# brunoasm/varKoder

Measured on AMD Instinct MI355X. Metric: Gbases/s for `varKoder image` k=7, 150 bp reads, higher is better.
Workload: dtype u32

## Files before the change

varkoder_amd/csrc/vk_count.h:

```cpp
#ifndef VK_COUNT_H
#define VK_COUNT_H

#include <hip/hip_runtime.h>

#include <cstdint>

#include "vk_lane.h"

namespace {

constexpr int kWaves = 16;
constexpr int kCountThreads = kWaves * 64;
constexpr int kPiece = 4096;
constexpr uint32_t kMaxBins = 16384;
#ifndef VK_K1_OCC
#define VK_K1_OCC 8
#endif
#ifndef VK_K1_PF
#define VK_K1_PF 2
#endif


__device__ __forceinline__ uint32_t nl_flags(uint32_t w) {
    uint32_t z = w ^ 0x0A0A0A0Au;
// ... 728 lines not shown
        const uint32_t pos = have ? static_cast<uint32_t>(__builtin_ctzll(m)) : 0u;
        m &= m - 1ull;
        const uint32_t ph = (lph + t) & 3u;
        const bool anchor = have && ph == 0u;
        if (have && ph == 1u) acc += static_cast<long long>(blk + pos);
        if (anchor) acc -= static_cast<long long>(blk + pos) + 1ll;
        const unsigned long long am = __ballot(anchor);
        if (am != 0ull) {
            const uint32_t na = static_cast<uint32_t>(__builtin_popcountll(am));
            if (nanch + na > cap) full = true;
            else if (anchor) seg[nanch + static_cast<uint32_t>(__builtin_popcountll(am & ((1ull << ln) - 1ull)))] = static_cast<uint32_t>(blk + pos);
            if (!full) nanch += na;
        }
        ++t;
    }
}


#ifdef VK_DIAG_NO_DSADD
#define VK_DSADD(a) "s_nop 0\n\t"
#else
#define VK_DSADD(a) "ds_add_u32 " a ", %17\n\t"
#endif
template <int K>
__device__ __forceinline__ void windows_lds1(uint32_t ch, uint32_t C, uint32_t ok, uint32_t lds_base,
                                             uint32_t& probe_addr, unsigned long long& probe_mask) {
    static_assert(2 * K + 2 <= 16, "paired extraction needs the field << 2 to fit 16 bits");
    constexpr uint32_t kMask4 = ((1u << (2 * K)) - 1u) << 2;
    const uint32_t one = 1u;
    uint32_t w = vkl::lshl_or(vkl::alignbit(ok, ok, 16u), 1u, ok);
#pragma unroll
    for (int half = 0; half < 2; ++half) {
        uint32_t a[8];
#pragma unroll
        for (int j = 0; j < 4; ++j) {
            const int i = 15 - 4 * half - j;
            const int plo = i - 8;
            const int o = 30 + 2 * (plo - K + 1);
            const int word = o >> 5, sh = o & 31;
            uint32_t x;
            if (word == 1) x = sh == 0 ? C : (C >> sh);
            else x = vkl::alignbit(C, ch, static_cast<uint32_t>(sh));
            a[2 * j] = (x & kMask4) + lds_base;
            a[2 * j + 1] = ((x >> 16) & kMask4) + lds_base;
        }
        unsigned long long m0, m1, m2, m3, m4, m5, m6, m7;
        const unsigned long long exec_in = __builtin_amdgcn_read_exec();
        asm volatile(
            "v_add_co_u32_e64 %0, %1, %0, %0\n\t"
            "v_add_co_u32_e64 %0, %2, %0, %0\n\t"
            "v_add_co_u32_e64 %0, %3, %0, %0\n\t"
            "v_add_co_u32_e64 %0, %4, %0, %0\n\t"
            "v_add_co_u32_e64 %0, %5, %0, %0\n\t"
            "v_add_co_u32_e64 %0, %6, %0, %0\n\t"
            "v_add_co_u32_e64 %0, %7, %0, %0\n\t"
            "v_add_co_u32_e64 %0, %8, %0, %0\n\t"
            "s_mov_b64 exec, %1\n\t" VK_DSADD("%9") 
            "s_mov_b64 exec, %2\n\t" VK_DSADD("%10") 
            "s_mov_b64 exec, %3\n\t" VK_DSADD("%11") 
            "s_mov_b64 exec, %4\n\t" VK_DSADD("%12") 
            "s_mov_b64 exec, %5\n\t" VK_DSADD("%13") 
            "s_mov_b64 exec, %6\n\t" VK_DSADD("%14") 
            "s_mov_b64 exec, %7\n\t" VK_DSADD("%15") 
            "s_mov_b64 exec, %8\n\t" VK_DSADD("%16") 
            "s_mov_b64 exec, %18"
            : "+v"(w), "=&s"(m0), "=&s"(m1), "=&s"(m2), "=&s"(m3), "=&s"(m4), "=&s"(m5), "=&s"(m6), "=&s"(m7)
            : "v"(a[0]), "v"(a[1]), "v"(a[2]), "v"(a[3]), "v"(a[4]), "v"(a[5]), "v"(a[6]), "v"(a[7]), "v"(one), "s"(exec_in)
            : "memory");
        if (half == 1) {
            probe_addr = a[7];
            probe_mask = m7;
        }
    }
}

struct GeneralState {
    uint32_t ctx_c, ctx_bad, pph, hot, tick;
    uint32_t nanch, full, sites;
};



template <int K, bool INDEX>
__device__ __attribute__((noinline)) GeneralState general_piece(uint4 q0, uint4 q1, uint4 q2, uint4 q3, GeneralState st,
                                                                uint32_t packed, uint32_t* hist, uint32_t hist_base,
                                                                uint32_t* iseg, uint32_t icap, uint32_t iblk) {
    const uint32_t flags = packed & 3u, ph0 = (packed >> 2) & 3u, ivalid = packed >> 4;
    const int lane = static_cast<int>(lane_now());
    const uint32_t d[16] = {q0.x, q0.y, q0.z, q0.w, q1.x, q1.y, q1.z, q1.w, q2.x, q2.y, q2.z, q2.w, q3.x, q3.y, q3.z, q3.w};
    const bool first = (flags & 1u) != 0u, has_pre = (flags & 2u) != 0u;
    uint32_t pph = st.pph;
    vkl::LaneBits lb;
    const uint32_t c = __any(vkl::has_non_ascii(d)) ? vkl::classify<false>(d, lb) : vkl::classify<true>(d, lb);
    const uint32_t incl = wave_inclusive_sum(c);
    const uint32_t total = lane_bcast(incl, 63);
    if (first) pph = has_pre ? ph0 - lane_bcast(c, 0) : 0u;
    const uint32_t lph = (pph + incl - c) & 3u;
    vkl::Mask128 seq;
    const bool degenerate = __any(c > 4u);
    uint32_t s_raw = 0;
    const bool four = !degenerate && __any(c > 3u);
    if (degenerate) seq = vkl::seq_mask_general(lb.NL, lph);
    else if (four) seq = vkl::seq_mask_fast4(lb.NL, lph, vkl::ones_below, vkl::ones_not_below, s_raw);
    else seq = vkl::seq_mask_count(lb.NL, lph);
    uint32_t bad[4], ok[4];
    vkl::bad_mask(lb, seq, bad);
    const uint32_t badh = wave_prev_lane(bad[3], st.ctx_bad);
    const uint32_t ch = wave_prev_lane(lb.C[3], st.ctx_c);
    st.ctx_bad = lane_bcast(bad[3], 63);
    st.ctx_c = lane_bcast(lb.C[3], 63);
    vkl::ok_mask<K>(badh, bad, ok);
    if (first && lane == 0 && has_pre) { ok[0] = 0u; ok[1] = 0u; ok[2] = 0u; ok[3] = 0u; }
    if constexpr (INDEX) {
        const bool mine = !(first && lane == 0 && has_pre);
        uint32_t mlo, mhi;
        {
            uint32_t v[8];
#pragma unroll
            for (int j = 0; j < 8; ++j) v[j] = vkl::udot4(nl_flags(d[2 * j + 1]), 0x80402010u, vkl::udot4(nl_flags(d[2 * j]), 0x08040201u, 0u));
            mlo = (v[0] >> 7) | (v[1] << 1) | (v[2] << 9) | (v[3] << 17);
            mhi = (v[4] >> 7) | (v[5] << 1) | (v[6] << 9) | (v[7] << 17);
        }
        bool full = false;
        long long unused = 0;
        uint32_t nanch = st.nanch;
        index_block(mlo, mhi, lph, static_cast<uint64_t>(iblk) + 64u * static_cast<uint32_t>(lane), mine, iseg, icap, nanch, full, unused);
        st.nanch = nanch;
        st.full = full ? 1u : 0u;
        uint32_t sites = 0;
        const int vb = static_cast<int>(ivalid) - 64 * lane;
#pragma unroll
        for (int g = 0; g < 4; ++g) {
            const int vg = vb - 16 * g;
            const uint32_t inside = vg >= 16 ? 0xFFFFFFFFu : (vg <= 0 ? 0u : ((1u << (2 * vg)) - 1u));
            sites += vkl::popc(seq.w[g] & ~lb.NL[g] & inside & 0x55555555u);
        }
        st.sites = mine ? sites : 0u;
    }
    uint32_t pa;
    unsigned long long pm;
    uint32_t still = 0;
    uint32_t tick = st.tick & 0x7FFFFFFFu;
    if (st.hot == 0u) windows_lds<K>(ch, lb.C, ok, hist_base, pa, pm);
    else {
        ++tick;
        uint4* const xb = reinterpret_cast<uint4*>(hist + (1u << (2 * K))) + (threadIdx.x >> 6) * 64u;
        still = windows_lds_hot<K>(ch, lb.C, ok, hist, hist_base, lane, (st.tick >> 31) == 0u || (tick & 7u) == 0u, pa, pm, xb);
    }
    st.hot = (still != 0u || probe_low_complexity(pa, pm, tick)) ? 1u : 0u;
    st.tick = (tick & 0x7FFFFFFFu) | (still == 2u ? 0x80000000u : 0u);
    st.pph = pph + total;
    __builtin_amdgcn_s_waitcnt(0xC07F);
    return st;
}

constexpr uint32_t kSetAside = 6;
constexpr uint32_t kSetAsideBatch = 21;

template <int K, bool INDEX>
__global__ __launch_bounds__(kCountThreads, 8) void vk_aside_kernel(const uint8_t* __restrict__ fastq, const uint64_t* __restrict__ offs,
                                                                     const uint64_t* __restrict__ lens, uint32_t nsamples, uint32_t parts,
                                                                     uint32_t* __restrict__ hist_out, const uint32_t* __restrict__ aside,
                                                                     uint32_t aside_cap, const uint32_t* __restrict__ aside_n, IndexParams ip,
                                                                     uint32_t upb) {
    typedef uint32_t u32x4 __attribute__((ext_vector_type(4)));
    constexpr uint32_t NCODE = 1u << (2 * K);
    constexpr bool LDSH = NCODE <= kMaxBins;
    __shared__ uint32_t lhist[LDSH ? NCODE : 1];
    __shared__ uint32_t any_list;
    const uint32_t ablocks = (parts + upb - 1u) / upb;
    const uint32_t smp = blockIdx.x / ablocks;
    const uint32_t part0 = (blockIdx.x % ablocks) * upb, part1 = part0 + upb < parts ? part0 + upb : parts;
    const uint32_t tid = threadIdx.x;
    const uint32_t wave = static_cast<uint32_t>(__builtin_amdgcn_readfirstlane(static_cast<int>(tid >> 6)));
    if (tid == 0) any_list = 0u;
    __syncthreads();
    {
        uint32_t any = 0u;
        for (uint32_t part = part0; part < part1; ++part) any |= aside_n[(smp * parts + part) * kWaves + wave];
        if (any != 0u && (tid & 63u) == 0u) any_list = 1u;
    }
    __syncthreads();
    if (any_list == 0u) return;
    if constexpr (LDSH) {
        for (uint32_t i = tid; i < NCODE; i += kCountThreads) lhist[i] = 0u;
        __syncthreads();
    }
    const uint32_t lhist_base = static_cast<uint32_t>(reinterpret_cast<uintptr_t>((__attribute__((address_space(3))) uint32_t*)lhist));
    const uint8_t* sbase = fastq + offs[smp];
    uint32_t* hist = hist_out + static_cast<uint64_t>(smp) * NCODE;
    const uint32_t lane = tid & 63u;
    const uint32_t ent = lane / 3u, j = lane - 3u * ent;
    for (uint32_t part = part0; part < part1; ++part) {
    const uint32_t unit = smp * parts + part;
    const uint32_t gw = unit * kWaves + wave;
    const uint32_t naside = aside_n[gw];
    const WaveRange wr = wave_range(lens[smp], parts, part, static_cast<int>(wave));
    const uint64_t o0 = wr.w0 != 0 ? wr.w0 - 64 : 0;
    const uint64_t span = wr.w1 - o0;
    const __amdgpu_buffer_rsrc_t rsrc = __builtin_amdgcn_make_buffer_rsrc(
        const_cast<uint8_t*>(sbase + o0), 0, static_cast<int>((span + 15) & ~15ull), 0x00020000);
    const uint32_t* list = aside + static_cast<uint64_t>(gw) * aside_cap;
    uint32_t* iseg = nullptr;
    uint32_t icap = 0, nanch = 0, isites = 0;
    bool ifull = false;
    if constexpr (INDEX) {
        iseg = ip.anchors + index_segment(ip, smp, wr.w0, part, static_cast<int>(wave));
        icap = static_cast<uint32_t>(index_segment_cap(wr.w1 - wr.w0));
        nanch = ip.count[gw];
    }
    for (uint32_t at = 0; at < naside; at += kSetAsideBatch) {
        const uint32_t n = naside - at < kSetAsideBatch ? naside - at : kSetAsideBatch;
        const bool live = ent < n;
        const uint32_t w = live ? list[at + ent] : 0u;
        const uint32_t off = live ? ((w >> 3) - 1u + j) * 64u : 0xFFFFFF00u;
        const u32x4 a = __builtin_amdgcn_raw_buffer_load_b128(rsrc, off, 0, 0);
        const u32x4 b = __builtin_amdgcn_raw_buffer_load_b128(rsrc, off, 16, 0);
        const u32x4 c4 = __builtin_amdgcn_raw_buffer_load_b128(rsrc, off, 32, 0);
        const u32x4 e4 = __builtin_amdgcn_raw_buffer_load_b128(rsrc, off, 48, 0);
        const uint32_t d[16] = {a.x, a.y, a.z, a.w, b.x, b.y, b.z, b.w, c4.x, c4.y, c4.z, c4.w, e4.x, e4.y, e4.z, e4.w};
        vkl::LaneBits lb;
        const uint32_t c = vkl::classify<false>(d, lb);
        const uint32_t cprev = wave_prev_lane(c, 0u);
        const uint32_t lph = ((w & 3u) + (j == 0u ? 0u - c : (j == 2u ? cprev : 0u))) & 3u;
        vkl::Mask128 seq;
        uint32_t s_raw = 0;
        if (__any(c > 4u)) seq = vkl::seq_mask_general(lb.NL, lph);
        else seq = vkl::seq_mask_fast4(lb.NL, lph, vkl::ones_below, vkl::ones_not_below, s_raw);
        uint32_t bad[4], ok[4];
        vkl::bad_mask(lb, seq, bad);
        const uint32_t badh = wave_prev_lane(bad[3], 0x55555555u);
        const uint32_t ch = wave_prev_lane(lb.C[3], 0u);
        vkl::ok_mask<K>(badh, bad, ok);
        constexpr uint32_t kBack = (1u << (2 * (K - 1))) - 1u;
        if (!live || j == 0u) { ok[0] = 0u; ok[1] = 0u; ok[2] = 0u; ok[3] = 0u; }
        if (j == 1u && (w & 4u) != 0u) ok[0] &= ~kBack;
        if (j == 2u) { ok[0] &= kBack; ok[1] = 0u; ok[2] = 0u; ok[3] = 0u; }
        if constexpr (LDSH) {
            uint32_t pa;
            unsigned long long pm;
            windows_lds<K>(ch, lb.C, ok, lhist_base, pa, pm);
        } else {
            vkl::windows<K>(ch, lb.C, ok, [&](uint32_t field4) { atomicAdd(&hist[pair_reverse(field4 >> 2, K)], 1u); }, [] {});
        }
        if constexpr (INDEX) {
            const bool mine = live && j == 1u;
            uint32_t mlo, mhi;
            {
                uint32_t v[8];
#pragma unroll
                for (int jj = 0; jj < 8; ++jj) v[jj] = vkl::udot4(nl_flags(d[2 * jj + 1]), 0x80402010u, vkl::udot4(nl_flags(d[2 * jj]), 0x08040201u, 0u));
                mlo = (v[0] >> 7) | (v[1] << 1) | (v[2] << 9) | (v[3] << 17);
                mhi = (v[4] >> 7) | (v[5] << 1) | (v[6] << 9) | (v[7] << 17);
            }
            long long unused = 0;
            index_block(mlo, mhi, lph, o0 + static_cast<uint64_t>(off), mine, iseg, icap, nanch, ifull, unused);
            if (mine) {
#pragma unroll
                for (int g = 0; g < 4; ++g) isites += vkl::popc(seq.w[g] & ~lb.NL[g] & 0x55555555u);
            }
        }
    }
    if constexpr (INDEX) {
        const uint32_t tot = lane_bcast(wave_inclusive_sum(isites), 63);
        if (lane == 0u && naside != 0u) {
            ip.count[gw] = nanch;
            if (tot != 0u) atomicAdd(&ip.sites[smp], static_cast<unsigned long long>(tot));
            if (ifull) atomicOr(&ip.overflow[smp], 1u);
        }
    }
    }
    if constexpr (LDSH) {
        __builtin_amdgcn_s_waitcnt(0xC07F);
        __syncthreads();
        for (uint32_t code = tid; code < NCODE; code += kCountThreads) {
            const uint32_t v = lhist[pair_reverse(code, K)];
            if (v) atomicAdd(&hist[code], v);
        }
    }
}

struct PullParams {
    uint32_t* words;
    uint32_t helpers;
};
__host__ __device__ constexpr size_t pull_words(uint32_t nsamples) { return 2 + 2 * static_cast<size_t>(nsamples); }

template <int K, bool INDEX, bool PULL = false>
__global__ __launch_bounds__(kCountThreads, VK_K1_OCC) void vk_count_dense_kernel(
    const uint8_t* __restrict__ fastq, const uint64_t* __restrict__ offs,
    const uint64_t* __restrict__ lens, uint32_t nsamples, uint32_t parts,
    uint32_t* __restrict__ hist_out, uint32_t* __restrict__ wavephase, int atomic_flush,
    uint32_t* __restrict__ aside, uint32_t aside_cap, uint32_t* __restrict__ aside_n, IndexParams ip, PullParams pull) {
    static_assert(!(PULL && INDEX), "the index launch keeps its static split");
    constexpr uint32_t NCODE = 1u << (2 * K);
    static_assert(NCODE <= kMaxBins, "LDS histogram too large");
    struct DenseLds {
        uint32_t hist[NCODE];
        uint4 xbuf[kWaves][64];
    };
    __shared__ __attribute__((aligned(16))) DenseLds dlds;
    uint32_t (&hist)[NCODE] = dlds.hist;
    uint4 (&xbuf)[kWaves][64] = dlds.xbuf;

    const int tid = threadIdx.x;
    const int lane = tid & 63;
    const int wave = __builtin_amdgcn_readfirstlane(tid >> 6);
    constexpr uint32_t kNoSample = 0xFFFFFFFFu;
    auto add0 = [&](uint32_t* p, uint32_t v) __attribute__((always_inline)) {
        uint32_t r = 0;
        if (lane == 0) r = atomicAdd(p, v);
        return static_cast<uint32_t>(__builtin_amdgcn_readfirstlane(static_cast<int>(r)));
    };
    uint32_t smp = blockIdx.x / parts;
    do {
    if constexpr (PULL) {
        uint32_t* const word = reinterpret_cast<uint32_t*>(&xbuf[0][0]);
        if (wave == 0) {
            uint32_t got = add0(&pull.words[0], 1u);
            if (got >= nsamples) {
                got = kNoSample;
                const uint64_t tickets = static_cast<uint64_t>(nsamples) * pull.helpers;
                uint32_t t;
                do {
                    t = add0(&pull.words[1], 1u);
                    if (t < tickets) {
                        const uint32_t s = nsamples - 1u - t % nsamples;
                        if (add0(&pull.words[2u + s], 0u) < parts * kWaves) got = s;
                    }
                } while (t < tickets && got == kNoSample);
            }
            if (lane == 0) *word = got;
        }
        __syncthreads();
        smp = static_cast<uint32_t>(__builtin_amdgcn_readfirstlane(static_cast<int>(*word)));
    }
    if (!PULL || smp != kNoSample) {

    for (uint32_t i = tid; i < NCODE; i += kCountThreads) hist[i] = 0u;
    __syncthreads();

    uint32_t chunk = PULL ? add0(&pull.words[2u + smp], 1u) : 0u;
    if (!PULL || chunk < parts * kWaves) do {
    const uint32_t part = PULL ? chunk / kWaves : blockIdx.x % parts;
    const int cwave = PULL ? static_cast<int>(chunk % kWaves) : wave;
    const uint32_t unit = smp * parts + part;
    const WaveRange wr = wave_range(lens[smp], parts, part, cwave);
    uint32_t ph_start = 0, ph_end = 0, general_pieces = 0, aside_count = 0, anchors = 0;
    if (!wr.empty) {
        const uint32_t hist_base = static_cast<uint32_t>(reinterpret_cast<uintptr_t>(
            (__attribute__((address_space(3))) uint32_t*)hist));
        uint4* const xb = &xbuf[wave][0];
        const uint8_t* sbase = reinterpret_cast<const uint8_t*>(uniform64(reinterpret_cast<uint64_t>(fastq + offs[smp])));
        const uint64_t len = uniform64(lens[smp]), w0 = uniform64(wr.w0), w1 = uniform64(wr.w1);
        const uint32_t ph0 = (w0 != 0) ? sync_phase(sbase, w0, len, reinterpret_cast<uint64_t*>(xb), lane) : 0u;
        ph_start = ph0;
        const bool has_pre = w0 != 0;
        const uint64_t o0 = has_pre ? w0 - 64 : 0;
        const uint64_t span = w1 - o0;
        const uint32_t npieces = static_cast<uint32_t>((span + kPiece - 1) / kPiece);
        const uint32_t tail_bytes = static_cast<uint32_t>(span % kPiece);
        typedef uint32_t u32x4 __attribute__((ext_vector_type(4)));
        const __amdgpu_buffer_rsrc_t rsrc = __builtin_amdgcn_make_buffer_rsrc(
            const_cast<uint8_t*>(sbase + o0), 0, static_cast<int>((span + 15) & ~15ull), 0x00020000);
        uint4 r0, r1, r2, r3;
        auto load_piece = [&](uint32_t piece) {
            const uint32_t soff = piece * static_cast<uint32_t>(kPiece);
            const uint32_t lane64 = lane_now() << 6;
            const u32x4 a = __builtin_amdgcn_raw_buffer_load_b128(rsrc, lane64, soff, 0);
            const u32x4 b = __builtin_amdgcn_raw_buffer_load_b128(rsrc, lane64, soff + 16u, 0);
            const u32x4 c = __builtin_amdgcn_raw_buffer_load_b128(rsrc, lane64, soff + 32u, 0);
            const u32x4 d = __builtin_amdgcn_raw_buffer_load_b128(rsrc, lane64, soff + 48u, 0);
            r0 = make_uint4(a.x, a.y, a.z, a.w);
            r1 = make_uint4(b.x, b.y, b.z, b.w);
            r2 = make_uint4(c.x, c.y, c.z, c.w);
            r3 = make_uint4(d.x, d.y, d.z, d.w);
        };
        auto clip_granule = [](uint4& v, int n) {
            if (n >= 16) return;
            uint32_t w[4] = {v.x, v.y, v.z, v.w};
#pragma unroll
            for (int d = 0; d < 4; ++d) {
                const int kb = n - 4 * d;
                w[d] &= kb >= 4 ? 0xFFFFFFFFu : (kb <= 0 ? 0u : ((1u << (8 * kb)) - 1u));
            }
            v = make_uint4(w[0], w[1], w[2], w[3]);
        };

        uint32_t ctx_c = 0u, ctx_bad = 0x55555555u;
        uint32_t pph = 0;
        uint32_t npend = 0;
        bool hot = false;
        uint32_t tick = 0;
        uint32_t ngeneral = 0;
        uint32_t* const alist = aside + (static_cast<uint64_t>(unit) * kWaves + static_cast<uint32_t>(cwave)) * aside_cap;
        uint32_t naside = 0;
        uint32_t aside63 = 0;
        uint32_t* const iseg = INDEX ? ip.anchors + uniform64(index_segment(ip, smp, w0, part, cwave)) : nullptr;
        const uint32_t icap = INDEX ? static_cast<uint32_t>(index_segment_cap(w1 - w0)) : 0u;
        uint32_t nanch = 0, nsite = 0;
        bool ifull = false;

        auto round_count = [&](uint32_t n, uint4 q, bool probe, bool full = true) __attribute__((always_inline)) {
#ifdef VK_DIAG_NO_HEAVY
            asm volatile("" :: "v"(q.x), "v"(q.y), "v"(q.z), "v"(q.w));
            return;
#endif
            uint32_t C, bad, SEQ;
            vkl::classify_granule_note(q.x, q.y, q.z, q.w, C, bad, SEQ);
            if constexpr (INDEX) nsite += vkl::popc(SEQ & 0x55555555u);
            uint32_t badh = ctx_bad, ch = ctx_c;
            if (full) {
                uint32_t nb, nc;
                asm("s_nop 1\n\t"
                    "v_mov_b32_dpp %0, %4 wave_shr:1 row_mask:0xf bank_mask:0xf\n\t"
                    "v_mov_b32_dpp %1, %5 wave_shr:1 row_mask:0xf bank_mask:0xf\n\t"
                    "v_mov_b32_dpp %2, %4 wave_ror:1 row_mask:0xf bank_mask:0xf\n\t"
                    "v_mov_b32_dpp %3, %5 wave_ror:1 row_mask:0xf bank_mask:0xf"
                    : "+v"(badh), "+v"(ch), "=&v"(nb), "=&v"(nc) : "v"(bad), "v"(C));
                ctx_bad = nb;
                ctx_c = nc;
            } else {
                badh = wave_prev_lane(bad, ctx_bad);
                ch = wave_prev_lane(C, ctx_c);
                ctx_bad = static_cast<uint32_t>(__builtin_amdgcn_readlane(static_cast<int>(bad), static_cast<int>(n - 1u)));
                ctx_c = static_cast<uint32_t>(__builtin_amdgcn_readlane(static_cast<int>(C), static_cast<int>(n - 1u)));
            }
            const uint32_t ok = vkl::ok_mask1<K>(badh, bad);
            uint32_t pa;
            unsigned long long pm;
            windows_lds1<K>(ch, C, ok, hist_base, pa, pm);
            if (probe) hot = probe_low_complexity(pa, pm, tick);
        };
        auto flush = [&]() __attribute__((always_inline)) {
            uint4 q = make_uint4(0x0A0A0A0Au, 0x0A0A0A0Au | vkl::kGranuleEnd, 0x0A0A0A0Au, 0x0A0A0A0Au);
            const uint32_t ln = lane_now();
            if (ln < npend) q = xb[ln];
            round_count(npend, q, true, false);
            npend = 0u;
        };

        load_piece(0);
#ifdef VK_STAMPS
        unsigned long long st_wait = 0, st_all = 0, st_t0 = 0, st_t1 = 0, st_prev = 0;
        VK_STAMP(st_prev);
#endif
#ifndef VK_DIAG_K1_NO_PACE
        [[maybe_unused]] const uint32_t pace_at = npieces - (npieces >> 2);
        if constexpr (!PULL) __builtin_amdgcn_s_setprio(1);
#endif
        for (uint32_t it = 0; it < npieces; ++it) {
#ifndef VK_DIAG_K1_NO_PACE
            if (!PULL && it == pace_at) __builtin_amdgcn_s_setprio(0);
#endif
#ifdef VK_STAMPS
            VK_STAMP(st_t0);
            asm volatile("s_waitcnt vmcnt(0)" ::: "memory");
            VK_STAMP(st_t1);
            st_wait += st_t1 - st_t0;
            st_all += st_t0 - st_prev;
            st_prev = st_t0;
#endif
            if (it + 1 == npieces && (tail_bytes & 15u) != 0u) {
                uint32_t tb = tail_bytes;
                asm volatile("" : "+s"(tb));
                const int n = static_cast<int>(tb) - static_cast<int>(lane_now() << 6);
                clip_granule(r0, n);
                clip_granule(r1, n - 16);
                clip_granule(r2, n - 32);
                clip_granule(r3, n - 48);
            }
            const uint4 q0 = r0, q1 = r1, q2 = r2, q3 = r3;
            const uint32_t d[16] = {q0.x, q0.y, q0.z, q0.w, q1.x, q1.y, q1.z, q1.w,
                                    q2.x, q2.y, q2.z, q2.w, q3.x, q3.y, q3.z, q3.w};
            bool fast = it != 0 && it + 1 != npieces && !hot && !__any(vkl::ascii_or(d) != 0u);
            uint32_t total = 0, s = 64, e = 64;
            if (fast) {
                uint32_t mlo, mhi;
                vkl::newline_mask64(d, mlo, mhi);
                const uint32_t c = vkl::popc(mlo) + vkl::popc(mhi);
                const uint32_t incl = wave_inclusive_sum(c);
                total = lane_bcast(incl, 63);
                const uint32_t dn = (c - incl + (1u - pph)) & 3u;
                uint32_t s_raw;
                const bool plain = vkl::seq_span_note(mlo, mhi, c, dn, s, e, s_raw);
                const unsigned long long am = __builtin_amdgcn_ballot_w64(!plain);
                if (am != 0ull) {
                    const uint32_t na = static_cast<uint32_t>(__builtin_popcountll(am));
#ifdef VK_DIAG_NO_ASIDE
                    if (true) {
#else
                    if (na > kSetAside || naside + na > aside_cap) {
#endif
                        fast = false;
                    } else {
                        if (!plain) {
                            const uint32_t ln = lane_now();
                            const uint32_t below = __builtin_amdgcn_mbcnt_hi(static_cast<uint32_t>(am >> 32), __builtin_amdgcn_mbcnt_lo(static_cast<uint32_t>(am), 0u));
                            const bool before = ln == 0u ? aside63 != 0u : ((am >> (ln - 1u)) & 1ull) != 0ull;
                            const __amdgpu_buffer_rsrc_t arsrc = __builtin_amdgcn_make_buffer_rsrc(alist, 0, static_cast<int>(aside_cap * 4u), 0x00020000);
                            __builtin_amdgcn_raw_buffer_store_b32(((it * 64u + ln) << 3) | (before ? 4u : 0u) | ((1u - dn) & 3u), arsrc, (naside + below) * 4u, 0, 0);
                            s = 0u;
                            e = 0u;
                        }
                        naside = static_cast<uint32_t>(__builtin_amdgcn_readfirstlane(static_cast<int>(naside + na)));
                    }
                }
                aside63 = fast ? static_cast<uint32_t>(am >> 63) : 0u;
                if constexpr (INDEX) {
                    const bool has = fast && plain && s_raw >= 1u && s_raw <= 64u;
                    const unsigned long long hm = __ballot(has);
                    if (hm != 0ull) {
                        const uint32_t nh = static_cast<uint32_t>(__builtin_popcountll(hm));
                        const uint32_t ln = lane_now();
                        if (nanch + nh > icap) ifull = true;
                        else if (has) {
                            const __amdgpu_buffer_rsrc_t irsrc = __builtin_amdgcn_make_buffer_rsrc(iseg, 0, static_cast<int>(icap * 4u), 0x00020000);
                            const uint32_t rank = __builtin_amdgcn_mbcnt_hi(static_cast<uint32_t>(hm >> 32), __builtin_amdgcn_mbcnt_lo(static_cast<uint32_t>(hm), 0u));
                            __builtin_amdgcn_raw_buffer_store_b32(static_cast<uint32_t>(o0) + it * static_cast<uint32_t>(kPiece) + 64u * ln + s_raw - 1u,
                                                                  irsrc, (nanch + rank) * 4u, 0, 0);
                        }
                        if (!ifull) nanch += nh;
                    }
                }
            }
            if (!fast) aside63 = 0u;
            uint32_t mode = 0u, tot = 0u;
            uint4 qa = make_uint4(0u, 0u, 0u, 0u), qb = qa;
            if (!fast) {
                if (npend != 0u) flush();
                ++ngeneral;
                GeneralState gs;
                gs.ctx_c = static_cast<uint32_t>(__builtin_amdgcn_readfirstlane(static_cast<int>(ctx_c)));
                gs.ctx_bad = static_cast<uint32_t>(__builtin_amdgcn_readfirstlane(static_cast<int>(ctx_bad)));
                gs.pph = pph; gs.hot = hot ? 1u : 0u; gs.tick = tick;
                gs.nanch = nanch; gs.full = 0u; gs.sites = 0u;
                const uint32_t valid = (it + 1 == npieces && tail_bytes != 0u) ? tail_bytes : static_cast<uint32_t>(kPiece);
#ifdef VK_DIAG_NO_GENERAL
                {
                    const uint32_t c = nl_count16(q0) + nl_count16(q1) + nl_count16(q2) + nl_count16(q3);
                    const uint32_t incl = wave_inclusive_sum(c);
                    if (it == 0) gs.pph = has_pre ? ph0 - lane_bcast(c, 0) : 0u;
                    gs.pph += lane_bcast(incl, 63);
                    gs.ctx_bad = 0x55555555u;
                }
#else
                gs = general_piece<K, INDEX>(q0, q1, q2, q3, gs, (it == 0 ? 1u : 0u) | (has_pre ? 2u : 0u) | (ph0 << 2) | (valid << 4),
                                             hist, hist_base, iseg, icap, static_cast<uint32_t>(o0) + it * static_cast<uint32_t>(kPiece));
#endif
                if constexpr (INDEX) {
                    nanch = static_cast<uint32_t>(__builtin_amdgcn_readfirstlane(static_cast<int>(gs.nanch)));
                    if (__builtin_amdgcn_readfirstlane(static_cast<int>(gs.full)) != 0) ifull = true;
                    nsite += gs.sites;
                }
                ctx_c = static_cast<uint32_t>(__builtin_amdgcn_readfirstlane(static_cast<int>(gs.ctx_c)));
                ctx_bad = static_cast<uint32_t>(__builtin_amdgcn_readfirstlane(static_cast<int>(gs.ctx_bad)));
                pph = static_cast<uint32_t>(__builtin_amdgcn_readfirstlane(static_cast<int>(gs.pph)));
                hot = __builtin_amdgcn_readfirstlane(static_cast<int>(gs.hot)) != 0;
                tick = static_cast<uint32_t>(__builtin_amdgcn_readfirstlane(static_cast<int>(gs.tick)));
                total = 0u;
            } else {
                const uint32_t gs = vkl::span_first(s), n = ((vkl::umin(e, 63u) + 16u) >> 4) - gs;
                const uint32_t incl = wave_inclusive_sum(n);
                tot = npend + lane_bcast(incl, 63);
                const uint32_t mine0 = npend + incl - n;
                const uint32_t first = mine0 - gs;
                constexpr uint32_t kNoRound = 0xFFFFFFFFu;
                const uint32_t xb_base = static_cast<uint32_t>(reinterpret_cast<uintptr_t>((__attribute__((address_space(3))) uint4*)xb));
                uint32_t rd[5], ad[5];
                uint32_t minebits;
                asm("v_bfm_b32 %0, %1, %2" : "=v"(minebits) : "v"(n), "v"(gs));
#pragma unroll
                for (uint32_t g = 0; g < 4; ++g) {
                    const uint32_t place = first + g;
                    uint32_t own;
                    asm("v_bfe_i32 %0, %1, %2, 1" : "=v"(own) : "v"(minebits), "n"(g));
                    rd[g] = (place >> 6) | ~own;
                    ad[g] = vkl::lshl_add_s(place & 63u, 4, xb_base);
                }
                const bool has_s = (s & 15u) != 0u;
                const uint32_t pnote = has_s ? mine0 : (e < 64u ? mine0 + n - 1u : 0xFFFFFFFFu);
                rd[4] = pnote >> 6;
                ad[4] = vkl::lshl_add_s(pnote & 63u, 4, xb_base);
                const uint32_t note_lo = vkl::note_spread((s | e) & 15u), note_hi = has_s ? 0u : vkl::kGranuleEnd;
                const uint32_t rounds = tot >> 6;
                typedef uint32_t u32x4 __attribute__((ext_vector_type(4)));
                typedef uint32_t u32x2 __attribute__((ext_vector_type(2)));
                auto put = [&](uint32_t r) __attribute__((always_inline)) {
                    const u32x4 g0 = {r0.x, r0.y, r0.z, r0.w}, g1 = {r1.x, r1.y, r1.z, r1.w};
                    const u32x4 g2 = {r2.x, r2.y, r2.z, r2.w}, g3 = {r3.x, r3.y, r3.z, r3.w};
                    const u32x2 nt = {note_lo, note_hi};
                    unsigned long long m0, m1, m2, m3, m4;
                    const unsigned long long exec_in = __builtin_amdgcn_read_exec();
                    asm volatile(
                        "v_cmp_eq_u32_e64 %0, %5, %15\n\t"
                        "v_cmp_eq_u32_e64 %1, %6, %15\n\t"
                        "v_cmp_eq_u32_e64 %2, %7, %15\n\t"
                        "v_cmp_eq_u32_e64 %3, %8, %15\n\t"
                        "v_cmp_eq_u32_e64 %4, %9, %15\n\t"
                        "s_mov_b64 exec, %0\n\tds_write_b128 %10, %16\n\t"
                        "s_mov_b64 exec, %1\n\tds_write_b128 %11, %17\n\t"
                        "s_mov_b64 exec, %2\n\tds_write_b128 %12, %18\n\t"
                        "s_mov_b64 exec, %3\n\tds_write_b128 %13, %19\n\t"
                        "s_mov_b64 exec, %4\n\tds_or_b64 %14, %20\n\t"
                        "s_mov_b64 exec, %21"
                        : "=&s"(m0), "=&s"(m1), "=&s"(m2), "=&s"(m3), "=&s"(m4)
                        : "v"(rd[0]), "v"(rd[1]), "v"(rd[2]), "v"(rd[3]), "v"(rd[4]),
                          "v"(ad[0]), "v"(ad[1]), "v"(ad[2]), "v"(ad[3]), "v"(ad[4]), "s"(r),
                          "v"(g0), "v"(g1), "v"(g2), "v"(g3), "v"(nt), "s"(exec_in)
                        : "memory");
                };
                uint32_t r = 0u;
                for (; r + 2u < rounds; ++r) {
                    put(r);
                    const uint4 q = xb[lane];
                    round_count(64u, q, false);
                }
                if (rounds >= 2u) {
                    put(r);
                    qa = xb[lane];
                    ++r;
                    mode = 2u;
                }
                if (rounds >= 1u) {
                    put(r);
                    qb = xb[lane];
                    ++r;
                    if (mode == 0u) mode = 1u;
                }
                put(r);
            }
            if (it + 1 < npieces) load_piece(it + 1);
            if (mode == 2u) round_count(64u, qa, false);
            if (mode != 0u) round_count(64u, qb, true);
            npend = tot & 63u;
            pph += total;
        }
        ph_end = pph & 3u;
        general_pieces = ngeneral < 0xFFFFFFu ? ngeneral : 0xFFFFFFu;
        aside_count = naside;
#ifdef VK_DIAG_ASIDE_INLINE
        if constexpr (!INDEX) {
            __builtin_amdgcn_s_waitcnt(0x0F70);
            const uint32_t* list = aside + static_cast<uint64_t>(unit * kWaves + static_cast<uint32_t>(cwave)) * aside_cap;
            const uint32_t ulane = static_cast<uint32_t>(lane);
            const uint32_t ent = ulane / 3u, j = ulane - 3u * ent;
            for (uint32_t at = 0; at < naside; at += kSetAsideBatch) {
                const uint32_t n = naside - at < kSetAsideBatch ? naside - at : kSetAsideBatch;
                const bool live = ent < n;
                const uint32_t w = live ? list[at + ent] : 0u;
                const uint32_t off = live ? ((w >> 3) - 1u + j) * 64u : 0xFFFFFF00u;
                const u32x4 a = __builtin_amdgcn_raw_buffer_load_b128(rsrc, off, 0, 0);
                const u32x4 b = __builtin_amdgcn_raw_buffer_load_b128(rsrc, off, 16, 0);
                const u32x4 c4 = __builtin_amdgcn_raw_buffer_load_b128(rsrc, off, 32, 0);
                const u32x4 e4 = __builtin_amdgcn_raw_buffer_load_b128(rsrc, off, 48, 0);
                const uint32_t d[16] = {a.x, a.y, a.z, a.w, b.x, b.y, b.z, b.w, c4.x, c4.y, c4.z, c4.w, e4.x, e4.y, e4.z, e4.w};
                vkl::LaneBits lb;
                const uint32_t c = vkl::classify<false>(d, lb);
                const uint32_t cprev = wave_prev_lane(c, 0u);
                const uint32_t lph = ((w & 3u) + (j == 0u ? 0u - c : (j == 2u ? cprev : 0u))) & 3u;
                vkl::Mask128 seq;
                uint32_t s_raw = 0;
                if (__any(c > 4u)) seq = vkl::seq_mask_general(lb.NL, lph);
                else seq = vkl::seq_mask_fast4(lb.NL, lph, vkl::ones_below, vkl::ones_not_below, s_raw);
                uint32_t bad[4], ok[4];
                vkl::bad_mask(lb, seq, bad);
                const uint32_t badh = wave_prev_lane(bad[3], 0x55555555u);
                const uint32_t ch = wave_prev_lane(lb.C[3], 0u);
                vkl::ok_mask<K>(badh, bad, ok);
                constexpr uint32_t kBack = (1u << (2 * (K - 1))) - 1u;
                if (!live || j == 0u) { ok[0] = 0u; ok[1] = 0u; ok[2] = 0u; ok[3] = 0u; }
                if (j == 1u && (w & 4u) != 0u) ok[0] &= ~kBack;
                if (j == 2u) { ok[0] &= kBack; ok[1] = 0u; ok[2] = 0u; ok[3] = 0u; }
                uint32_t pa;
                unsigned long long pm;
                windows_lds<K>(ch, lb.C, ok, hist_base, pa, pm);
            }
        }
#endif
        if constexpr (INDEX) {
            anchors = nanch;
            const uint32_t tot = lane_bcast(wave_inclusive_sum(nsite), 63);
            if (lane == 0) {
                if (tot != 0u) atomicAdd(&ip.sites[smp], static_cast<unsigned long long>(tot));
                if (ifull || len >= (1ull << 32)) atomicOr(&ip.overflow[smp], 1u);
            }
        }
        __builtin_amdgcn_s_waitcnt(0xC07F);
#ifdef VK_STAMPS
        if (lane == 0 && (blockIdx.x & 63u) == 0u) {
            atomicAdd(&g_vk_stamps[5], st_wait);
            atomicAdd(&g_vk_stamps[6], st_all);
            atomicAdd(&g_vk_stamps[7], static_cast<unsigned long long>(npieces));
        }
#endif
    }
    if (lane == 0) {
        wavephase[unit * kWaves + cwave] = wr.empty ? 0x80u : (0x40u | ph_start | (ph_end << 2) | (general_pieces << 8));
        aside_n[unit * kWaves + cwave] = aside_count;
        if constexpr (INDEX) ip.count[unit * kWaves + cwave] = anchors;
    }
    if constexpr (PULL) chunk = add0(&pull.words[2u + smp], 1u);
    } while (PULL && chunk < parts * kWaves);

    __syncthreads();
    uint32_t* out = hist_out + static_cast<uint64_t>(smp) * NCODE;
    for (uint32_t code = tid; code < NCODE; code += kCountThreads) {
        const uint32_t v = hist[pair_reverse(code, K)];
        if (atomic_flush) {
            if (v) atomicAdd(&out[code], v);
        } else {
            out[code] = v;
        }
    }
    if constexpr (PULL)
        if (tid == 0) atomicAdd(&pull.words[2u + nsamples + smp], 1u);
    }
    } while (PULL && smp != kNoSample);
}

constexpr uint32_t kPackHasPre = 0x80000000u;
constexpr uint32_t kPackBlock = 256;

struct PackParams {
    uint32_t* c;
    uint32_t* m;
    const uint64_t* base;
    uint32_t* count;
};

__device__ __forceinline__ uint64_t pack_segment(const PackParams& pk, uint32_t smp, uint32_t part, int wave, uint64_t w0) {
    return pk.base[smp] + (w0 >> 4) + 8ull * (static_cast<uint64_t>(part) * kWaves + static_cast<uint32_t>(wave));
}

constexpr uint32_t kQueues = 16;
constexpr uint32_t kQueueBytes = 256;
constexpr uint32_t kQueueShift = 6;
constexpr uint32_t kBlockBytes = 64;
constexpr uint32_t kQueueBlocks = kQueueBytes / kBlockBytes;
constexpr uint32_t kRunBytes = 4096;
constexpr uint32_t kRunBlocks = kRunBytes / kBlockBytes;
constexpr uint32_t kDrainAt = 2 * kBlockBytes;
constexpr uint32_t kDrainAtCalm = 3 * kBlockBytes;
constexpr uint32_t kNoRun = 0x100;

struct BucketParams {
    uint32_t* cursors;
    uint32_t* hdrs;
    uint8_t* arena;
    uint32_t* bucket_hist;
    uint32_t* bsize;
    uint32_t* order;
    uint32_t* wide;
    uint32_t runs_cap;
    uint32_t force_wide;
    uint32_t* qfirst;
    uint32_t* qlist;
    uint32_t* preg;
    uint32_t* preg_n;
    uint32_t preg_shift;
    uint32_t parts;
};

constexpr uint32_t kLdsCnt = 0;
constexpr uint32_t kLdsRun = kLdsCnt + kWaves * kQueues * 4;
constexpr uint32_t kLdsUsed = kLdsRun + kWaves * kQueues * 4;
constexpr uint32_t kLdsScratch = kLdsUsed + kWaves * kQueues * 4;
constexpr uint32_t kLdsBelow = kLdsScratch + kWaves * 64;
constexpr uint32_t kLdsAbove = kLdsBelow + 66 * 16;
constexpr uint32_t kLdsQueues = 8192;
constexpr uint32_t kLdsXchg = kLdsQueues + kWaves * kQueues * kQueueBytes;
constexpr uint32_t kLdsBucketBytes = kLdsXchg + kWaves * 64 * 8;
constexpr uint32_t kLdsPool = kLdsAbove + 66 * 16;
constexpr uint32_t kPoolRuns = 16;
constexpr uint32_t kLdsSync = kLdsPool + kWaves * 8;
constexpr uint32_t kLdsCntP = kLdsSync + 24;
static_assert(kLdsCntP + 256 * 4 <= kLdsQueues, "LDS layout");
constexpr uint32_t kQuadBuckets = 256;
static_assert(kQuadBuckets == kWaves * kQueues, "a wave drains sixteen of its workgroup's queues");
static_assert(2 * kLdsBucketBytes <= 160 * 1024, "two bucket workgroups per CU");

template <int K>
__device__ __forceinline__ uint32_t entry_raw(uint32_t q, uint32_t idx_and_type) {
    constexpr uint32_t LB = 2 * K - 4;
    const uint32_t idx = idx_and_type & ((1u << LB) - 1u);
    if ((idx_and_type >> LB) == 0u) return (q << LB) | idx;
    return (idx & ((1u << (LB - 2)) - 1u)) | (q << (LB - 2)) | ((idx >> (LB - 2)) << (2 * K - 2));
}

template <int K>
// ... 1187 lines not shown
```

varkoder_amd/csrc/vk_lane.h:

```cpp
#ifndef VK_LANE_H
#define VK_LANE_H

#include <stdint.h>

#if defined(__HIPCC__)
#define VKL_FN __host__ __device__ __forceinline__
#else
#define VKL_FN inline
#endif

namespace vkl {

VKL_FN uint32_t perm(uint32_t hi, uint32_t lo, uint32_t sel) {
#if defined(__HIP_DEVICE_COMPILE__)
    return __builtin_amdgcn_perm(hi, lo, sel);
#else
    uint64_t pool = (static_cast<uint64_t>(hi) << 32) | lo;
    uint32_t r = 0;
    for (int i = 0; i < 4; ++i) {
        uint32_t s = (sel >> (8 * i)) & 7u;
        r |= static_cast<uint32_t>((pool >> (8 * s)) & 0xFFu) << (8 * i);
    }
    return r;
#endif
// ... 172 lines not shown
    r[0] &= m.w[0]; r[1] &= m.w[1]; r[2] &= m.w[2]; r[3] &= m.w[3];
    const uint32_t p3 = first_newline(r);
    const uint32_t lo = 0xFFu | (p1 << 8) | (p2 << 16) | (p3 << 24);
    const uint32_t pr = alignbit(64u, lo, 8u * d);
    const uint32_t s = ((pr & 0xFFu) + 1u) & 0xFFu;
    const uint32_t e = (pr >> 8) & 0xFFu;
    s_raw = s;
    const Mask128 ms = above(umin(s, 64u)), me = below(umin(e, 64u));
    Mask128 out;
    for (int g = 0; g < 4; ++g) out.w[g] = me.w[g] & ms.w[g];
    return out;
}

template <typename Below, typename Above>
VKL_FN Mask128 seq_mask_fast(const uint32_t NL[4], uint32_t lph, Below below, Above above) {
    uint32_t s_raw;
    return seq_mask_fast(NL, lph, below, above, s_raw);
}

VKL_FN uint32_t rep_slots(uint32_t v) {
#if defined(__HIP_DEVICE_COMPILE__)
    const uint32_t r = __umul24(v, 0x555555u);
    return r | (r << 8);
#else
    return v * 0x55555555u;
#endif
}

VKL_FN Mask128 seq_mask_count(const uint32_t NL[4], uint32_t lph) {
    const uint32_t want = rep_slots((1u - lph) & 3u);
    Mask128 out;
    uint32_t before = 0;
    for (int g = 0; g < 4; ++g) {
        uint32_t x = NL[g];
        x += x << 2;
        x += x << 4;
        x += x << 8;
        x += x << 16;
        if (g) x += rep_slots(before);
        before += popc(NL[g]);
        const uint32_t z = x ^ want;
        out.w[g] = ~(z | (z >> 1)) & 0x55555555u;
    }
    return out;
}

template <typename Below, typename Above>
VKL_FN Mask128 seq_mask_fast4(const uint32_t NL[4], uint32_t lph, Below below, Above above, uint32_t& s_raw) {
    const uint32_t d = (1u - lph) & 3u;
    const uint32_t p1 = first_newline(NL);
    Mask128 m = above(umin(p1 + 1u, 64u));
    uint32_t r[4] = {NL[0] & m.w[0], NL[1] & m.w[1], NL[2] & m.w[2], NL[3] & m.w[3]};
    const uint32_t p2 = first_newline(r);
    m = above(umin(p2 + 1u, 64u));
    r[0] &= m.w[0]; r[1] &= m.w[1]; r[2] &= m.w[2]; r[3] &= m.w[3];
    const uint32_t p3 = first_newline(r);
    m = above(umin(p3 + 1u, 64u));
    r[0] &= m.w[0]; r[1] &= m.w[1]; r[2] &= m.w[2]; r[3] &= m.w[3];
    const uint32_t p4 = first_newline(r);
    const uint32_t lo = 0xFFu | (p1 << 8) | (p2 << 16) | (p3 << 24);
    const uint32_t hi = p4 | (64u << 8);
    const uint32_t pr = alignbit(hi, lo, 8u * d);
    const uint32_t s = ((pr & 0xFFu) + 1u) & 0xFFu;
    const uint32_t e = (pr >> 8) & 0xFFu;
    s_raw = s;
    const Mask128 ms = above(umin(s, 64u)), me = below(umin(e, 64u));
    const Mask128 m2 = above(d == 0u ? umin(p4 + 1u, 64u) : 64u);
    Mask128 out;
    for (int g = 0; g < 4; ++g) out.w[g] = (me.w[g] & ms.w[g]) | m2.w[g];
    return out;
}

VKL_FN uint32_t sample_hash(uint64_t seed, uint64_t anchor) {
    uint32_t h = static_cast<uint32_t>(anchor) ^ static_cast<uint32_t>(seed);
    h += static_cast<uint32_t>(anchor >> 32) * 0x9E3779B1u + static_cast<uint32_t>(seed >> 32);
    h ^= h >> 16; h *= 0x85EBCA6Bu;
    h ^= h >> 13; h *= 0xC2B2AE35u;
    h ^= h >> 16;
    return h;
}

VKL_FN bool sample_take(uint64_t seed, uint64_t anchor, uint64_t threshold) {
    return static_cast<uint64_t>(sample_hash(seed, anchor)) < threshold;
}

VKL_FN uint32_t sample_strings_general(const uint32_t NL[4], uint32_t lph, uint64_t base, uint64_t seed,
                                       uint64_t threshold, uint32_t first[4], uint32_t inc[4], uint32_t& last_take,
                                       uint32_t& last_anchor) {
    uint32_t cur = lph & 3u, anchors = 0, take = 0;
    last_take = 0;
    last_anchor = 0;
#if defined(__HIP_DEVICE_COMPILE__)
#pragma unroll
#endif
    for (int g = 0; g < 4; ++g) {
        uint32_t f = 0, n = 0;
        const uint32_t nl = NL[g];
#if defined(__HIP_DEVICE_COMPILE__)
#pragma nounroll
#endif
        for (uint32_t b = 0; b < 32; b += 2) {
            if (anchors == 0) f |= 3u << b;
            else if (take) n |= 3u << b;
            if ((nl >> b) & 1u) {
                if (cur == 0u) {
                    ++anchors;
                    take = sample_take(seed, base + 16u * static_cast<uint32_t>(g) + (b >> 1), threshold) ? 1u : 0u;
                    last_take = take;
                    last_anchor = 16u * static_cast<uint32_t>(g) + (b >> 1);
                }
                cur = (cur + 1u) & 3u;
            }
        }
        first[g] = f;
        inc[g] = n;
    }
    return anchors;
}

constexpr uint32_t kBreakLength = 500;
template <int K>
VKL_FN void break_stretches(uint32_t r, uint32_t& q1, uint32_t& lo2, uint32_t& hi2) {
    q1 = r <= static_cast<uint32_t>(K - 2) ? static_cast<uint32_t>(K - 1) - r : 0u;
    lo2 = umin(kBreakLength - r, 64u);
    hi2 = umin(lo2 + static_cast<uint32_t>(K - 1), 64u);
}

VKL_FN Mask128 ones_not_below(uint32_t q) {
    Mask128 m = ones_below(q);
    for (int g = 0; g < 4; ++g) m.w[g] = ~m.w[g];
    return m;
}

VKL_FN Mask128 seq_mask_general(const uint32_t NL[4], uint32_t lph) {
    Mask128 out;
    uint32_t cur = lph & 3u;
    for (int g = 0; g < 4; ++g) {
        uint32_t acc = 0;
        const uint32_t nl = NL[g];
#if defined(__HIP_DEVICE_COMPILE__)
#pragma nounroll
#endif
        for (uint32_t b = 0; b < 32; b += 2) {
            acc |= (cur == 1u ? 3u : 0u) << b;
            cur = (cur + ((nl >> b) & 1u)) & 3u;
        }
        out.w[g] = acc;
    }
    return out;
}

VKL_FN void bad_mask(const LaneBits& lb, const Mask128& seq, uint32_t bad[4]) {
    for (int g = 0; g < 4; ++g) bad[g] = (lb.IV[g] | ~seq.w[g]) & 0x55555555u;
}

template <int K>
VKL_FN void ok_mask(uint32_t badh, const uint32_t bad[4], uint32_t ok[4]) {
    uint32_t w[5] = {badh, bad[0], bad[1], bad[2], bad[3]};
    int cover = 1;
#if defined(__HIP_DEVICE_COMPILE__)
#pragma unroll
#endif
    for (int step = 0; step < 4; ++step) {
        if (cover < K) {
            const int shp = cover < K - cover ? cover : K - cover;
            const uint32_t sh = 2u * static_cast<uint32_t>(shp);
            for (int i = 4; i >= 1; --i) w[i] |= alignbit(w[i], w[i - 1], 32u - sh);
            w[0] |= w[0] << sh;
            cover += shp;
        }
    }
    for (int g = 0; g < 4; ++g) ok[g] = ~w[g + 1] & 0x55555555u;
}

template <int K, typename Emit, typename Hook>
VKL_FN void windows(uint32_t ch, const uint32_t C[4], const uint32_t ok[4], Emit emit, Hook after_group) {
    const uint32_t v[5] = {ch, C[0], C[1], C[2], C[3]};
    constexpr uint32_t kMask4 = ((1u << (2 * K)) - 1u) << 2;
#if defined(__HIP_DEVICE_COMPILE__)
#pragma unroll
#endif
    for (int g = 0; g < 4; ++g) {
        uint32_t w = ok[g] | (alignbit(ok[g], ok[g], 16u) << 1);
#if defined(__HIP_DEVICE_COMPILE__)
#pragma unroll
#endif
        for (int i = 15; i >= 8; --i) {
            const int plo = 16 * g + i - 8, phi = 16 * g + i;
            const int o = 30 + 2 * (plo - K + 1);
            const int word = o >> 5, sh = o & 31;
            if (2 * K + 2 <= 16) {
                uint32_t x;
                if (sh == 0) x = v[word];
                else if (word == 4) x = v[4] >> sh;
                else x = alignbit(v[word + 1], v[word], static_cast<uint32_t>(sh));
                const bool take_lo = __builtin_add_overflow(w, w, &w);
                if (take_lo) emit(x & kMask4);
                const bool take_hi = __builtin_add_overflow(w, w, &w);
                if (take_hi) emit((x >> 16) & kMask4);
            } else {
                const int o2 = o + 16, word2 = o2 >> 5, sh2 = o2 & 31;
                const bool take_lo = __builtin_add_overflow(w, w, &w);
                if (take_lo) {
                    const uint32_t x = (sh + 2 * K + 2 <= 32) ? (v[word] >> sh)
                                                               : alignbit(v[word + 1], v[word], static_cast<uint32_t>(sh));
                    emit(x & kMask4);
                }
                const bool take_hi = __builtin_add_overflow(w, w, &w);
                if (take_hi) {
                    const uint32_t x = (sh2 + 2 * K + 2 <= 32) ? (v[word2] >> sh2)
                                                                : alignbit(v[word2 + 1], v[word2], static_cast<uint32_t>(sh2));
                    emit(x & kMask4);
                }
            }
        }
        after_group();
    }
}


VKL_FN uint32_t udot4(uint32_t a, uint32_t b, uint32_t c) {
#if defined(__HIP_DEVICE_COMPILE__)
    return __builtin_amdgcn_udot4(a, b, c, false);
#else
    uint32_t r = c;
    for (int i = 0; i < 4; ++i) r += ((a >> (8 * i)) & 0xFFu) * ((b >> (8 * i)) & 0xFFu);
    return r;
#endif
}

VKL_FN uint32_t ascii_or(const uint32_t d[16]) {
    uint32_t o = 0;
    for (int i = 0; i < 16; i += 2) o |= d[i] | d[i + 1];
    return o & 0x80808080u;
}

VKL_FN void newline_mask64(const uint32_t d[16], uint32_t& lo, uint32_t& hi) {
    uint32_t v[8];
#if defined(__HIP_DEVICE_COMPILE__)
#pragma unroll
#endif
    for (int k = 0; k < 8; ++k) {
        const uint32_t f0 = xor_add_k(d[2 * k], 0x75757575u, 0x01010101u) & 0x80808080u;
        const uint32_t f1 = xor_add_k(d[2 * k + 1], 0x75757575u, 0x01010101u) & 0x80808080u;
        v[k] = udot4(f1, 0x80402010u, udot4(f0, 0x08040201u, 0u));
    }
    lo = (v[0] >> 7) | (v[1] << 1) | (v[2] << 9) | (v[3] << 17);
    hi = (v[4] >> 7) | (v[5] << 1) | (v[6] << 9) | (v[7] << 17);
}

VKL_FN uint32_t first_bit64(uint32_t lo, uint32_t hi) {
    return umin(umin(ffbl(lo), ffbl(hi) | 32u), 64u);
}

VKL_FN bool seq_span(uint32_t lo, uint32_t hi, uint32_t c, uint32_t lph, uint32_t& s, uint32_t& e, uint32_t& s_raw) {
    const uint32_t dn = (1u - lph) & 3u;
    const uint32_t p1 = first_bit64(lo, hi);
    const uint32_t lo1 = lo & (lo - 1u), hi1 = lo ? hi : (hi & (hi - 1u));
    const uint32_t p2 = first_bit64(lo1, hi1);
    const uint32_t cand = 0xFFu | (p1 << 8) | (p2 << 16) | (64u << 24);
    const uint32_t pr = alignbit(64u, cand, 8u * dn);
    s_raw = (pr + 1u) & 0xFFu;
    s = umin(s_raw, 64u);
    e = (pr >> 8) & 0xFFu;
    const bool both = (s >> 4) == (e >> 4) && (s & 15u) != 0u;
    const bool two = dn == 2u && (s & 15u) != 0u && (p1 >> 4) == (p2 >> 4);
    return c <= (dn >= 2u ? 2u : 3u) && !both && !two;
}

VKL_FN bool seq_span(uint32_t lo, uint32_t hi, uint32_t c, uint32_t lph, uint32_t& s, uint32_t& e) {
    uint32_t s_raw;
    return seq_span(lo, hi, c, lph, s, e, s_raw);
}

VKL_FN uint32_t span_first(uint32_t s) { return s >> 4; }
VKL_FN uint32_t span_last(uint32_t e) { return umin(e, 63u) >> 4; }
VKL_FN uint32_t span_count(uint32_t s, uint32_t e) { return s < 64u ? span_last(e) - span_first(s) + 1u : 0u; }

constexpr uint32_t kGranuleStartTag = 0x80u;
VKL_FN bool span_starts_inside(uint32_t s) { return s < 64u && (s & 15u) != 0u; }

VKL_FN void classify_granule(uint32_t a0, uint32_t a1, uint32_t a2, uint32_t a3, bool starts_inside,
                             uint32_t& Cout, uint32_t& IVout, uint32_t& SEQout) {
    constexpr uint32_t kLutLo = 0x41204020u, kLutHi = 0x42202053u;
    const uint32_t p01l = perm(a1, a0, 0x05010400u), p01h = perm(a1, a0, 0x07030602u);
    const uint32_t p23l = perm(a3, a2, 0x05010400u), p23h = perm(a3, a2, 0x07030602u);
    const uint32_t T[4] = {perm(p23l, p01l, 0x05040100u), perm(p23l, p01l, 0x07060302u),
                           perm(p23h, p01h, 0x05040100u), perm(p23h, p01h, 0x07060302u)};
    uint32_t C = 0, IV = 0, NL = 0;
#if defined(__HIP_DEVICE_COMPILE__)
#pragma unroll
#endif
    for (int j = 0; j < 4; ++j) {
        const uint32_t t = T[j];
        const uint32_t L = perm(kLutHi, kLutLo, t & 0x07070707u);
        const uint32_t x = xor_and_k(L, t, 0xD8D8D8D8u);
        C = j == 0 ? (x & 0x03030303u) : lshl_or(x & 0x03030303u, 2 * j, C);
        const uint32_t nz = x + 0x7C7C7C7Cu;
        const uint32_t eq = xor_add_k(t, 0x75757575u, 0x01010101u);
        IV = j == 0 ? ((nz >> 7) & 0x01010101u) : and_or_k(nz >> (7 - 2 * j), 0x01010101u << (2 * j), IV);
        NL = j == 0 ? ((eq >> 7) & 0x01010101u) : and_or_k(eq >> (7 - 2 * j), 0x01010101u << (2 * j), NL);
    }
    const uint32_t low = (NL - 1u) & ~NL;
    Cout = C;
    IVout = IV;
    SEQout = starts_inside ? ~((low << 2) | 3u) : low;
// ... 126 lines not shown
```

Measured before the change: 2480.

## Let first and last pieces of a chunk take the fast path in non-index mode

The count loop used to force the first and last piece of each chunk through the general path. A new noinline helper now rebuilds the k-mer context and line phase from the 64-byte granule just before the chunk. The fast path then masks out lanes outside the chunk (the pre-granule lane and lanes past the tail), and a final flush drains any pending set-aside work. The goal is to drop the slower general processing at chunk edges, at the cost of an extra granule read and a function call per chunk, plus more complex edge handling.

Result: no change. 2495, median of 6 (+0.6%).

```diff
diff --git a/varkoder_amd/csrc/vk_count.h b/varkoder_amd/csrc/vk_count.h
--- a/varkoder_amd/csrc/vk_count.h
+++ b/varkoder_amd/csrc/vk_count.h
@@ -904,6 +904,17 @@
     st.pph = pph + total;
     __builtin_amdgcn_s_waitcnt(0xC07F);
     return st;
+}
+
+typedef uint32_t vk_u32x4 __attribute__((ext_vector_type(4)));
+__device__ __attribute__((noinline)) vk_u32x4 chunk_start_context_at(const uint8_t* pre, uint32_t ph_w0) {
+    const uint4* p = reinterpret_cast<const uint4*>(pre);
+    const uint4 q0 = p[0], q1 = p[1], q2 = p[2], q3 = p[3];
+    const uint32_t d[16] = {q0.x, q0.y, q0.z, q0.w, q1.x, q1.y, q1.z, q1.w, q2.x, q2.y, q2.z, q2.w, q3.x, q3.y, q3.z, q3.w};
+    uint32_t ctx_c, ctx_bad;
+    const uint32_t c = vkl::chunk_start_context(d, ph_w0, ctx_c, ctx_bad);
+    const vk_u32x4 r = {ctx_c, ctx_bad, ph_w0 - c, 0u};
+    return r;
 }
 
 constexpr uint32_t kSetAside = 6;
@@ -1192,6 +1203,16 @@
             npend = 0u;
         };
 
+#ifndef VK_DIAG_K1_FIRST_GENERAL
+        if constexpr (!INDEX) {
+            if (has_pre) {
+                const u32x4 cx = chunk_start_context_at(sbase + o0, ph0);
+                ctx_c = cx.x;
+                ctx_bad = cx.y;
+                pph = static_cast<uint32_t>(__builtin_amdgcn_readfirstlane(static_cast<int>(cx.z)));
+            }
+        }
+#endif
         load_piece(0);
 #ifdef VK_STAMPS
         unsigned long long st_wait = 0, st_all = 0, st_t0 = 0, st_t1 = 0, st_prev = 0;
@@ -1225,7 +1246,14 @@
             const uint4 q0 = r0, q1 = r1, q2 = r2, q3 = r3;
             const uint32_t d[16] = {q0.x, q0.y, q0.z, q0.w, q1.x, q1.y, q1.z, q1.w,
                                     q2.x, q2.y, q2.z, q2.w, q3.x, q3.y, q3.z, q3.w};
-            bool fast = it != 0 && it + 1 != npieces && !hot && !__any(vkl::ascii_or(d) != 0u);
+#ifdef VK_DIAG_K1_FIRST_GENERAL
+            constexpr bool kFirstFast = false;
+#else
+            constexpr bool kFirstFast = !INDEX;
+#endif
+            const bool edge_ok = INDEX ? (it != 0 && it + 1 != npieces)
+                                       : ((kFirstFast || it != 0) && (it + 1 != npieces || (tail_bytes & 63u) == 0u));
+            bool fast = edge_ok && !hot && !__any(vkl::ascii_or(d) != 0u);
             uint32_t total = 0, s = 64, e = 64;
             if (fast) {
                 uint32_t mlo, mhi;
@@ -1233,9 +1261,23 @@
                 const uint32_t c = vkl::popc(mlo) + vkl::popc(mhi);
                 const uint32_t incl = wave_inclusive_sum(c);
                 total = lane_bcast(incl, 63);
-                const uint32_t dn = (c - incl + (1u - pph)) & 3u;
+                uint32_t dn = (c - incl + (1u - pph)) & 3u;
+                uint32_t cs = c;
+                if constexpr (!INDEX) {
+                    if (it == 0u || it + 1u == npieces) {
+                        const uint32_t ln = lane_now();
+                        const uint32_t lane_lo = (it == 0u && has_pre) ? 1u : 0u;
+                        const uint32_t lane_hi = (it + 1u == npieces && tail_bytes != 0u) ? tail_bytes >> 6 : 64u;
+                        if (ln < lane_lo || ln >= lane_hi) {
+                            mlo = 0u;
+                            mhi = 0u;
+                            cs = 0u;
+                            dn = 1u;
+                        }
+                    }
+                }
                 uint32_t s_raw;
-                const bool plain = vkl::seq_span_note(mlo, mhi, c, dn, s, e, s_raw);
+                const bool plain = vkl::seq_span_note(mlo, mhi, cs, dn, s, e, s_raw);
                 const unsigned long long am = __builtin_amdgcn_ballot_w64(!plain);
                 if (am != 0ull) {
                     const uint32_t na = static_cast<uint32_t>(__builtin_popcountll(am));
@@ -1388,6 +1430,8 @@
             npend = tot & 63u;
             pph += total;
         }
+        if constexpr (!INDEX)
+            if (npend != 0u) flush();
         ph_end = pph & 3u;
         general_pieces = ngeneral < 0xFFFFFFu ? ngeneral : 0xFFFFFFu;
         aside_count = naside;
diff --git a/varkoder_amd/csrc/vk_lane.h b/varkoder_amd/csrc/vk_lane.h
--- a/varkoder_amd/csrc/vk_lane.h
+++ b/varkoder_amd/csrc/vk_lane.h
@@ -348,6 +348,18 @@
 
 VKL_FN void bad_mask(const LaneBits& lb, const Mask128& seq, uint32_t bad[4]) {
     for (int g = 0; g < 4; ++g) bad[g] = (lb.IV[g] | ~seq.w[g]) & 0x55555555u;
+}
+
+VKL_FN uint32_t chunk_start_context(const uint32_t d[16], uint32_t ph_w0, uint32_t& ctx_c, uint32_t& ctx_bad) {
+    LaneBits lb;
+    const uint32_t c = classify<false>(d, lb);
+    const uint32_t lph = (ph_w0 - c) & 3u;
+    const Mask128 seq = c > 3u ? seq_mask_general(lb.NL, lph) : seq_mask_count(lb.NL, lph);
+    uint32_t bad[4];
+    bad_mask(lb, seq, bad);
+    ctx_c = lb.C[3];
+    ctx_bad = bad[3];
+    return c;
 }
 
 template <int K>
```
